# sadPororo/AD-YOLO

Hardware: AMD Instinct MI355X
Metric: train-step audio-sec/s (4ch, se-resnet34+adyolo) (higher is better)
Workload: dtype f32; 1 GPU; se-resnet34 + adyolo loss, synthetic 4ch 24kHz 60s clips, bs=64 per GPU, 12 classes, features+fwd+loss+bwd+allreduce+Adam; global_batch=64, parallelism=dp1

## Files before the change

ad-yolo_amd/_lib.py:

```python
import ctypes
import os

_HERE = os.path.dirname(os.path.abspath(__file__))
LIB_PATH = os.environ.get("ADYOLO_LIB") or os.path.join(_HERE, "libadyolo_hip.so")

P = ctypes.c_void_p
I = ctypes.c_int
L = ctypes.c_long
F = ctypes.c_float
U64 = ctypes.c_uint64

SIGNATURES = {
    "adyolo_abi_version": (I, []),
    "adyolo_last_error": (ctypes.c_char_p, []),
    "adyolo_feat_stft_mel": (I, [P] * 8 + [I, I] + [P] * 4 + [I, I, I, P]),
    "adyolo_feat_finish": (I, [P] * 4 + [I, I, I, P]),
    "adyolo_feat_gcc_phat": (I, [P] * 6 + [I, I, I, I, P]),
    "adyolo_nchw_to_nhwc8": (I, [P, P, I, I, I, I, P]),
    "adyolo_pack_w3x3": (I, [P, P, P, I, I, I, P]),
    "adyolo_conv3x3_tiles": (I, [I] * 3),
    "adyolo_conv3x3_fwd": (I, [P] * 13 + [I] * 7 + [P]),
    "adyolo_wino_pack_w": (I, [P, P, P, I, I, I, P]),
    "adyolo_wino_pack_many": (I, [P, I, I, I, P]),
    "adyolo_wino_tiles": (I, [I] * 3),
    "adyolo_wino_fwd": (I, [P] * 13 + [I] * 7 + [P]),
    "adyolo_wino4_pack_w": (I, [P, P, P, I, I, I, P]),
    "adyolo_wino4_pack_many": (I, [P, I, I, I, P]),
    "adyolo_wino4_tiles": (I, [I] * 3),
    "adyolo_wino4_fwd": (I, [P] * 13 + [I] * 7 + [P]),
    "adyolo_wino4_fwd_form": (I, [I] * 3),
    "adyolo_wino4_last_form": (I, []),
    "adyolo_set_switches": (I, [I]),
    "adyolo_wino4_wgrad_slabs": (I, [I] * 5),
    "adyolo_wino4_wgrad": (I, [P] * 7 + [I] * 6 + [P]),
    "adyolo_wino_wgrad_slabs": (I, [I] * 5),
    "adyolo_wino_wgrad": (I, [P] * 7 + [I] * 6 + [P]),
    "adyolo_conv3x3_wgrad_slabs": (I, [I] * 5),
    "adyolo_conv3x3_wgrad": (I, [P] * 6 + [I] * 6 + [P]),
    "adyolo_wgrad_plan": (I, [I] * 6 + [P]),
    "adyolo_conv_fwd_plan": (I, [I] * 9 + [P]),
    "adyolo_gemm": (I, [P] * 5 + [I] * 10 + [P]),
    "adyolo_gemm_plan": (I, [I] * 8 + [P, P, P]),
    "adyolo_gemm_batched": (I, [P] * 3 + [I] * 10 + [L] * 6 + [F, I, P]),
    "adyolo_colsum": (I, [P, P, P, I, I, I, I, P]),
    "adyolo_bn_stats": (I, [P] * 7 + [I, I, I, F, F, P]),
    "adyolo_bn_stats_tiles": (I, [P] * 11 + [I, I, I, I, F, F, P]),
    "adyolo_bn_eval_stats": (I, [P] * 4 + [I, F, P]),
    "adyolo_bn_scale_shift": (I, [P] * 6 + [I, P]),
    "adyolo_affine_nhwc": (I, [P] * 4 + [L, I, P]),
    "adyolo_bn_bwd_reduce": (I, [P] * 7 + [L, I, P]),
    "adyolo_bn_bwd_tiles": (I, [P, P, P, P, I, I, P]),
    "adyolo_bn_bwd_apply": (I, [P] * 12 + [L, I, I, F, P]),
    "adyolo_bn_persample": (I, [P, P, P, I, I, I, P]),
    "adyolo_bn_finish": (I, [P] * 10 + [I, I, I, F, F, P]),
    "adyolo_se_fc_fwd": (I, [P] * 10 + [I, I, I, I, P]),
    "adyolo_relu_mask_words": (L, [I, I, I]),
    "adyolo_se_tail_fwd": (I, [P] * 9 + [I, I, I, P]),
    "adyolo_se_tail_fwd_pool_ok": (I, [I, I, I]),
    "adyolo_se_tail_fwd_pool": (I, [P] * 9 + [I, I, I, I, P]),
    "adyolo_se_tail_bwd_reduce": (I, [P] * 9 + [I, I, I, P]),
    "adyolo_se_tail_bwd_tiles": (I, [P, P, P, I, I, I, P]),
    "adyolo_se_fc_bwd_words": (L, [I, I]),
    "adyolo_se_fc_bwd": (I, [P] * 16 + [I, I, I, I, P]),
    "adyolo_se_tail_bwd_apply": (I, [P] * 13 + [I, I, I, F, P]),
    "adyolo_se_tail_bwd_reduce_pooled": (I, [P] * 8 + [I, I, I, I, P]),
    "adyolo_se_tail_bwd_apply_pooled": (I, [P] * 13 + [I, I, I, I, F, P]),
    "adyolo_avgpool2_fwd": (I, [P, P, I, I, I, I, P]),
    "adyolo_avgpool2_bwd": (I, [P, P, I, I, I, I, P]),
    "adyolo_add": (I, [P, P, P, L, P]),
    "adyolo_mul": (I, [P, P, P, L, P]),
    "adyolo_scale_dev": (I, [P, P, P, L, P]),
    "adyolo_sap_fwd": (I, [P] * 5 + [I, I, I, P]),
    "adyolo_sap_bwd": (I, [P] * 8 + [I, I, I, P]),
    "adyolo_gru_fwd": (I, [P] * 6 + [I, I, P]),
    "adyolo_gru_bwd": (I, [P] * 6 + [I, I, P]),
    "adyolo_ln_tanh_fwd": (I, [P] * 4 + [L, I, F, P]),
    "adyolo_ln_tanh_bwd": (I, [P] * 8 + [L, I, F, P]),
    "adyolo_dropout_mask": (I, [P, L, F, U64, U64, P]),
    "adyolo_dropout_apply": (I, [P, P, L, F, U64, U64, P]),
    "adyolo_dropout_apply_dev": (I, [P, P, L, F, U64, U64, P, P]),
    "adyolo_counter_add": (I, [P, U64, P]),
    "adyolo_loss_workspace_words": (L, [I, I, I, I]),
    "adyolo_loss_fwd_bwd": (I, [P] * 6 + [I] * 7 + [P, P, F, F, F, F, P]),
    "adyolo_loss_phase": (I, [P] * 6 + [I] * 7 + [P, P, F, F, F, F, I, L, P]),
    "adyolo_loss_per_clip_workspace_words": (L, [I, I, I, I]),
    "adyolo_loss_per_clip": (I, [P] * 7 + [I] * 6 + [L, P, P, F, F, F, P]),
    "adyolo_loss_accumulate": (I, [P, P, I, P, P]),
    "adyolo_yolo_decode": (I, [P, P, L, I, I, I, I, F, F, F, P]),
    "adyolo_yolo_select_workspace_words": (L, [L, I, I]),
    "adyolo_yolo_select": (I, [P] * 4 + [L, I, I, F, F, F, F, I, P]),
    "adyolo_seld_score_workspace_words": (L, [L, I, I, I]),
    "adyolo_seld_score": (I, [P, I, L, P, L, I] + [P] * 5 + [I, I, I, I, ctypes.c_double, P, P, P, P]),
    "adyolo_act_fwd": (I, [P, P, L, I, I, P]),
    "adyolo_act_bwd": (I, [P, P, P, L, I, I, P]),
    "adyolo_seddoa_loss": (I, [P] * 5 + [L, I, I, I, F, F, P]),
    "adyolo_adpit_loss": (I, [P] * 5 + [L, I, P]),
    "adyolo_classwise_decode": (I, [P, P, L, I, I, P]),
    "adyolo_classwise_select_workspace_words": (L, [L, I, I]),
    "adyolo_classwise_select": (I, [P] * 4 + [L, I, I, F, F, P]),
    "adyolo_tta_merge_workspace_words": (L, [L, I]),
    "adyolo_tta_collect": (I, [P, L, P, P, P, P, P, L, I, I, I, I, ctypes.c_uint, P]),
    "adyolo_tta_merge": (I, [P, P, P, P, L, P, P, L, I, I, I, F, I, P]),
    "adyolo_conv_gemm": (I, [P, P, P, P] + [I] * 13 + [P]),
    "adyolo_conv_gemm_plan": (I, [I] * 13 + [P]),
    "adyolo_pack_wk": (I, [P, P, I, I, I, I, I, P]),
    "adyolo_maxpool3_fwd": (I, [P, P, P, I, I, I, I, P]),
    "adyolo_maxpool3_bwd": (I, [P, P, P, I, I, I, I, P]),
    "adyolo_affine_relu_nhwc": (I, [P] * 4 + [L, I, P]),
    "adyolo_relu_bwd": (I, [P, P, P, L, P]),
    "adyolo_axpby": (I, [P, P, P, F, F, L, P]),
    "adyolo_dropout_axpby": (I, [P, P, P, L, F, U64, U64, P, F, F, P]),
    "adyolo_swish_fwd": (I, [P, P, L, P]),
    "adyolo_swish_bwd": (I, [P, P, P, L, P]),
    "adyolo_glu_fwd": (I, [P, P, L, I, P]),
    "adyolo_glu_bwd": (I, [P, P, P, L, I, P]),
    "adyolo_dwconv3_fwd": (I, [P] * 4 + [I, I, I, I, I, P]),
    "adyolo_dwconv3_wgrad": (I, [P] * 6 + [I, I, I, I, P]),
    "adyolo_softmax_fwd": (I, [P, P, L, I, F, P]),
    "adyolo_softmax_bwd": (I, [P, P, P, L, I, F, P]),
# ... 93 lines not shown
```

ad-yolo_amd/csrc/norm.hip:

```cpp
#include "common.hpp"

namespace adyolo {

#ifndef ADYOLO_EW_NT
#define ADYOLO_EW_NT 3
#endif
__device__ __forceinline__ float4 ew_ld(const float4 *p) {
#if ADYOLO_EW_NT & 1
    const f32x4 v = __builtin_nontemporal_load(reinterpret_cast<const f32x4 *>(p));
    return make_float4(v[0], v[1], v[2], v[3]);
#else
    return *p;
#endif
}
__device__ __forceinline__ void ew_st(float4 *p, const float4 &v) {
#if ADYOLO_EW_NT & 2
    const f32x4 t = {v.x, v.y, v.z, v.w};
    __builtin_nontemporal_store(t, reinterpret_cast<f32x4 *>(p));
#else
    *p = v;
#endif
}


// ... 535 lines not shown
        ew_st(&dc4[i], o);
        if (dr4) dr4[i] = g;
    };
    if (INV) {
        load_params((int)threadIdx.x % c4n);
        const long step = (long)gridDim.x * 256 * EW_U;
        for (long i0 = (long)blockIdx.x * 256 * EW_U + threadIdx.x; i0 < hw4; i0 += step) {
            float4 d[EW_U], cv[EW_U];
            bool px[EW_U], py[EW_U], pz[EW_U], pw[EW_U];
#pragma unroll
            for (int u = 0; u < EW_U; ++u) {
                const long i = i0 + u * 256;
                if (i < hw4) {
                    if (POOLED) {
                        const int pix = (int)(i >> c4shift), y = pix / W, x = pix - y * W;
                        const float4 g4 = de4[(((size_t)(y >> 1) * (W >> 1) + (x >> 1)) << c4shift) + (i & (c4n - 1))];
                        d[u] = make_float4(0.25f * g4.x, 0.25f * g4.y, 0.25f * g4.z, 0.25f * g4.w);
                    } else {
                        d[u] = ew_ld(&de4[i]);
                    }
                    cv[u] = ew_ld(&c4[i]);
                    if (mask) {
                        mask_bits4(mask, base + i, px[u], py[u], pz[u], pw[u]);
                    } else {
                        const float4 ev = e4[i];
                        px[u] = ev.x > 0.f; py[u] = ev.y > 0.f; pz[u] = ev.z > 0.f; pw[u] = ev.w > 0.f;
                    }
                }
            }
#pragma unroll
            for (int u = 0; u < EW_U; ++u) {
                const long i = i0 + u * 256;
                if (i < hw4) {
                    one(i, d[u], cv[u], px[u], py[u], pz[u], pw[u]);
                    if (POOLED && deo4) ew_st(&deo4[i], d[u]);
                }
            }
        }
    } else {
        for (long i = (long)blockIdx.x * blockDim.x + threadIdx.x; i < hw4; i += (long)gridDim.x * blockDim.x) {
            load_params((int)(i % c4n));
            bool px, py, pz, pw;
            if (mask) {
                mask_bits4(mask, base + i, px, py, pz, pw);
            } else {
                const float4 ev = e4[i];
                px = ev.x > 0.f; py = ev.y > 0.f; pz = ev.z > 0.f; pw = ev.w > 0.f;
            }
            one(i, de4[i], c4[i], px, py, pz, pw);
        }
    }
}

__global__ __launch_bounds__(256) void avgpool2_fwd_kernel(const float *__restrict__ x, float *__restrict__ y,
                                                           int H, int W, int c4n, long total4) {
    const int Ho = H >> 1, Wo = W >> 1;
    for (long i = (long)blockIdx.x * blockDim.x + threadIdx.x; i < total4; i += (long)gridDim.x * blockDim.x) {
        const int cx = (int)(i % c4n);
        long p = i / c4n;
        const int wo = (int)(p % Wo);
        p /= Wo;
        const int ho = (int)(p % Ho);
        const long n = p / Ho;
        const float4 *src = reinterpret_cast<const float4 *>(x) + (((size_t)n * H + 2 * ho) * W + 2 * wo) * c4n + cx;
        const float4 a = ew_ld(src), b = ew_ld(src + c4n), c = ew_ld(src + (size_t)W * c4n), d = ew_ld(src + (size_t)W * c4n + c4n);
        reinterpret_cast<float4 *>(y)[i] = make_float4(0.25f * (a.x + b.x + c.x + d.x), 0.25f * (a.y + b.y + c.y + d.y),
                                                       0.25f * (a.z + b.z + c.z + d.z), 0.25f * (a.w + b.w + c.w + d.w));
    }
}
__global__ __launch_bounds__(256) void avgpool2_bwd_kernel(const float *__restrict__ dy, float *__restrict__ dx,
                                                           int H, int W, int c4n, long total4) {
    const int Ho = H >> 1, Wo = W >> 1;
    for (long i = (long)blockIdx.x * blockDim.x + threadIdx.x; i < total4; i += (long)gridDim.x * blockDim.x) {
        const int cx = (int)(i % c4n);
        long p = i / c4n;
        const int w = (int)(p % W);
        p /= W;
        const int h = (int)(p % H);
        const long n = p / H;
        const float4 g = reinterpret_cast<const float4 *>(dy)[(((size_t)n * Ho + (h >> 1)) * Wo + (w >> 1)) * c4n + cx];
        ew_st(&reinterpret_cast<float4 *>(dx)[i], make_float4(0.25f * g.x, 0.25f * g.y, 0.25f * g.z, 0.25f * g.w));
    }
}

static inline int ew_grid(long n4) {
    long g = (n4 + 255) / 256;
    return (int)(g > 8192 ? 8192 : (g < 1 ? 1 : g));
}
static inline bool chan_ok(int C) { return C >= 4 && C <= 1024 && (C % 4) == 0 && (256 % (C / 4)) == 0; }
static inline int pick_G(int N, int HW) {
    int G = 1024 / N;
    if (G < 1) G = 1;
    const int need = (HW + 63) / 64;
    if (G > need) G = need;
    return G;
}

}

using namespace adyolo;

extern "C" int adyolo_bn_stats(const float *x, float *ssum, float *mean, float *invstd, float *running_mean,
                               float *running_var, float *partial, int N, int HW, int C, float momentum, float eps,
                               void *stream) {
    ADYOLO_REQUIRE(x && mean && invstd && partial && N > 0 && HW > 0, ADYOLO_EINVAL, "bn_stats: bad arguments");
    ADYOLO_REQUIRE(chan_ok(C) && N <= 1024, ADYOLO_ENOSUP, "bn_stats: unsupported C=%d or N=%d", C, N);
// ... 258 lines not shown
    hipLaunchKernelGGL(se_fc_bwd_sample_kernel, dim3(N), dim3(256), 0, as_stream(stream), sg, sgx, ssum, gamma, beta,
                       mean, invstd, pooled, hid, s, w1, w2, dpool, part, HW, C, Cr);
    int rc = check_launch("se_fc_bwd_sample");
    if (rc) return rc;
    const long P = adyolo_se_fc_bwd_words(C, Cr);
    return adyolo_colsum(part, packed, colsum_ws, N, (int)P, (int)P, 0, stream);
}

extern "C" int adyolo_se_tail_bwd_apply(const float *de, const float *e, const uint64_t *mask, const float *c,
                                        const float *gamma, const float *mean, const float *invstd, const float *s,
                                        const float *dpool, const float *sdd, const float *sddx, float *dc, float *dr,
                                        int N, int HW, int C, float count_scale, void *stream) {
    ADYOLO_REQUIRE(de && (e || mask) && c && gamma && mean && invstd && s && dpool && sdd && sddx && dc && N > 0 &&
                       HW > 0 && C % 4 == 0 && count_scale >= 1.f,
                   ADYOLO_EINVAL, "se_tail_bwd_apply: bad arguments");
    const float inv_r = (float)(1.0 / ((double)N * (double)HW * (double)count_scale));
    const long hw4 = (long)HW * (C / 4);
    const bool inv = 256 % (C / 4) == 0;
    int gx = ew_grid(inv ? cdiv(hw4, (long)EW_U) : hw4);
    if ((long)gx * N > 16384) gx = (int)(16384 / N > 0 ? 16384 / N : 1);
    if (inv)
        hipLaunchKernelGGL(se_tail_bwd_apply_kernel<true>, dim3(gx, N), dim3(256), 0, as_stream(stream), de, e, c, gamma,
                           mean, invstd, s, dpool, sdd, sddx, dc, dr, reinterpret_cast<const unsigned long long *>(mask),
                           hw4, C / 4, 1.0f / (float)HW, inv_r);
    else
        hipLaunchKernelGGL(se_tail_bwd_apply_kernel<false>, dim3(gx, N), dim3(256), 0, as_stream(stream), de, e, c, gamma,
                           mean, invstd, s, dpool, sdd, sddx, dc, dr, reinterpret_cast<const unsigned long long *>(mask),
                           hw4, C / 4, 1.0f / (float)HW, inv_r);
    return check_launch("se_tail_bwd_apply");
}

extern "C" int adyolo_se_tail_bwd_apply_pooled(const float *dpooled, const uint64_t *mask, const float *c, const float *gamma,
                                               const float *mean, const float *invstd, const float *s, const float *dpool,
                                               const float *sdd, const float *sddx, float *dc, float *dr, float *de_out, int N,
                                               int H, int W, int C, float count_scale, void *stream) {
    ADYOLO_REQUIRE(dpooled && mask && c && gamma && mean && invstd && s && dpool && sdd && sddx && dc && N > 0 && H > 0 && W > 0 &&
                       count_scale >= 1.f,
                   ADYOLO_EINVAL, "se_tail_bwd_apply_pooled: bad arguments");
    ADYOLO_REQUIRE(adyolo_se_tail_fwd_pool_ok(H, W, C), ADYOLO_ENOSUP, "se_tail_bwd_apply_pooled: unsupported shape H=%d W=%d C=%d",
                   H, W, C);
    const int HW = H * W, c4n = C / 4;
    int c4shift = 0;
    while ((1 << c4shift) < c4n) ++c4shift;
    const float inv_r = (float)(1.0 / ((double)N * (double)HW * (double)count_scale));
    const long hw4 = (long)HW * c4n;
    int gx = ew_grid(cdiv(hw4, (long)EW_U));
    if ((long)gx * N > 16384) gx = (int)(16384 / N > 0 ? 16384 / N : 1);
    hipLaunchKernelGGL((se_tail_bwd_apply_kernel<true, true>), dim3(gx, N), dim3(256), 0, as_stream(stream), dpooled,
                       (const float *)nullptr, c, gamma, mean, invstd, s, dpool, sdd, sddx, dc, dr,
                       reinterpret_cast<const unsigned long long *>(mask), hw4, c4n, 1.0f / (float)HW, inv_r, W, c4shift, de_out);
    return check_launch("se_tail_bwd_apply_pooled");
}

extern "C" int adyolo_avgpool2_fwd(const float *x, float *y, int N, int H, int W, int C, void *stream) {
    ADYOLO_REQUIRE(x && y && N > 0 && H > 0 && W > 0 && H % 2 == 0 && W % 2 == 0 && C % 4 == 0, ADYOLO_EINVAL,
                   "avgpool2_fwd: H, W must be even and C %% 4 == 0");
    const long total4 = (long)N * (H / 2) * (W / 2) * (C / 4);
    hipLaunchKernelGGL(avgpool2_fwd_kernel, dim3(ew_grid(total4)), dim3(256), 0, as_stream(stream), x, y, H, W, C / 4,
                       total4);
    return check_launch("avgpool2_fwd");
}
extern "C" int adyolo_avgpool2_bwd(const float *dy, float *dx, int N, int H, int W, int C, void *stream) {
    ADYOLO_REQUIRE(dy && dx && N > 0 && H > 0 && W > 0 && H % 2 == 0 && W % 2 == 0 && C % 4 == 0, ADYOLO_EINVAL,
                   "avgpool2_bwd: H, W must be even and C %% 4 == 0");
    const long total4 = (long)N * H * W * (C / 4);
    hipLaunchKernelGGL(avgpool2_bwd_kernel, dim3(ew_grid(total4)), dim3(256), 0, as_stream(stream), dy, dx, H, W, C / 4,
                       total4);
    return check_launch("avgpool2_bwd");
}
```

ad-yolo_amd/functional.py:

```python
import os
from typing import NamedTuple

import torch

from . import ops

FUSE_BNBWD = os.environ.get("ADYOLO_FUSE_BNBWD", "1") != "0"
FUSE_POOL = os.environ.get("ADYOLO_FUSE_POOL", "1") != "0"
FUSE_POOL_BWD = os.environ.get("ADYOLO_FUSE_POOL_BWD", "1") != "0"


class BlockLink:

    def __init__(self):
        self.cc = self.mean2 = self.invstd2 = self.tiles = self.ebits = None
        self.affine = self.stem_bn = None
        self.prepooled = None


class BlockArgs(NamedTuple):
    bn1: object
    bn2: object
    bnd: object = None
    link_in: object = None
    link_out: object = None
    in_affine: tuple = None
    stem_holder: object = None
    packs: tuple = None
    pool_next: bool = False


def _c(t):
    return t if t.is_contiguous() else t.contiguous()


_CONST = {}


def _const(value, shape, device):
    key = (float(value), tuple(shape), str(device))
    t = _CONST.get(key)
    if t is None:
        t = torch.full(tuple(shape), float(value), dtype=torch.float32, device=device)
        _CONST[key] = t
    return t


class GradSink:

    def __init__(self):
        self.views = None
        self.notify = None
        self.step = 4

    def begin(self, flat, reducer=None):
        self.views = {p.data_ptr(): (i, p.grad) for i, p in enumerate(flat.params)}
        self.notify = reducer.notify if (reducer is not None and reducer.active) else None

    def end(self):
        self.views = self.notify = None

    def view(self, ptr, shape=None):
# ... 215 lines not shown
        if ctx.link_out is not None:
            link_out.cc, link_out.mean2, link_out.invstd2, link_out.tiles = cc, mean2, invstd2, None
            link_out.ebits = ebits
        ctx.training, ctx.pool, ctx.has_down = training, pool and not prepooled, wd is not None
        ctx.pool_out = (h, w_) if pool_out else None
        ctx.in_hw = (x.shape[1], x.shape[2])
        ctx.p_aff = p_aff
        ctx.stem_holder = args.stem_holder
        ctx.dgrad_packs = (wpk1d, wpk2d)
        ctx.ptrs = (w1.data_ptr(), g1.data_ptr(), b1.data_ptr(), w2.data_ptr(),
                    (fb2.data_ptr(), fw2.data_ptr(), fb1.data_ptr(), fw1.data_ptr(), b2.data_ptr(), g2.data_ptr()))
        ctx.wshapes = (tuple(w1.shape), tuple(w2.shape))
        ctx.down_ptrs = (wd.data_ptr(), gd.data_ptr(), bd.data_ptr(), tuple(wd.shape)) if wd is not None else None
        tensors = [p, a, scale1, shift1, cc, None if pool_out else e, ebits, g1, mean1, invstd1, g2, b2, mean2, invstd2, ssum2,
                   pooled, hid, s, fw1, fw2]
        names = ["p", "a", "scale1", "shift1", "cc", "e", "ebits", "g1", "mean1", "invstd1", "g2", "b2", "mean2", "invstd2",
                 "ssum2", "pooled", "hid", "s", "fw1", "fw2"]
        if wd is not None:
            tensors += [q, wd, gd, meand, invstdd]
            names += ["q", "wd", "gd", "meand", "invstdd"]
        ctx.saved_names = names
        ctx.save_for_backward(*tensors)
        return e

    @staticmethod
    def backward(ctx, de):
        if not ctx.training:
            raise NotImplementedError("backward through eval-mode BatchNorm is not part of the hot path")
        t = ctx.saved_tensors
        (p, a, scale1, shift1, cc, e, ebits, g1, mean1, invstd1, g2, b2, mean2, invstd2, ssum2, pooled, hid, s, fw1,
         fw2) = t[:20]
        wpk1d, wpk2d = ctx.dgrad_packs
        n, h, w_, cin = p.shape
        c = cc.shape[-1]
        de = _c(de)
        pooled_hw = None
        if ctx.pool_out is not None and FUSE_POOL_BWD:
            pooled_hw = ctx.pool_out
        elif ctx.pool_out is not None:
            de = ops.avgpool2_bwd(de, ctx.pool_out[0], ctx.pool_out[1])
        tiles = None
        if ctx.link_out is not None and ctx.link_out.tiles is not None:
            tiles, ctx.link_out.tiles = ctx.link_out.tiles, None
        pw1, pg1, pb1, pw2, pse = ctx.ptrs
        vse = SINK.span(pse)
        vw1, vw2 = SINK.view(pw1, ctx.wshapes[0]), SINK.view(pw2, ctx.wshapes[1])
        vg1, vb1 = SINK.view(pg1), SINK.view(pb1)
        sunk = vse is not None and vw1 is not None and vw2 is not None and vg1 is not None and vb1 is not None
        if not sunk:
            vse = vw1 = vw2 = vg1 = vb1 = None
        de_full = None
        if pooled_hw is not None and not ctx.has_down:
            de_full = torch.empty(n, pooled_hw[0], pooled_hw[1], c, dtype=torch.float32, device=de.device)
        dc, dr, dg2, db2, dfw1, dfb1, dfw2, dfb2 = ops.se_tail_bwd(de, e, cc, g2, b2, mean2, invstd2, ssum2, pooled,
                                                                   hid, s, fw1, fw2,
                                                                   want_dr=ctx.has_down, tile_stats=tiles,
                                                                   mask=ebits, packed_out=vse, pooled_hw=pooled_hw,
                                                                   de_out=de_full)
        if pooled_hw is not None:
            de = de_full
        dw2 = ops.conv3x3_wgrad(a, dc, c, in_affine=(scale1, shift1), out=vw2)
        if FUSE_BNBWD:
            dbb, st = ops.conv3x3(dc, wpk2d, c, want_stats=True, stat_bn=(a, mean1, invstd1))
            da, dg1, db1 = ops.bn_bwd(dbb, a, g1, mean1, invstd1, relu_mask=True, tile_stats=st, out_dgamma=vg1,
                                      out_dbeta=vb1)
        else:
            dbb = ops.conv3x3(dc, wpk2d, c)
            da, dg1, db1 = ops.bn_bwd(dbb, a, g1, mean1, invstd1, relu_mask=True, out_dgamma=vg1, out_dbeta=vb1)
        dw1 = ops.conv3x3_wgrad(p, da, cin, in_affine=ctx.p_aff, out=vw1)
        if sunk:
            SINK.done(*pse)
            SINK.done(pw2, pg1, pb1, pw1)
            dw1 = dg1 = db1 = dw2 = dg2 = db2 = dfw1 = dfb1 = dfw2 = dfb2 = None
        dwd = dgd = dbd = None
        if ctx.has_down:
            q, wd, gd, meand, invstdd = t[20:25]
            pwd, pgd, pbd, wdshape = ctx.down_ptrs
            vwd, vgd, vbd = SINK.view(pwd, (wdshape[0], wdshape[1])), SINK.view(pgd), SINK.view(pbd)
            dsunk = sunk and vwd is not None and vgd is not None and vbd is not None
            if not dsunk:
                vwd = vgd = vbd = None
            dq, dgd, dbd = ops.bn_bwd(dr, q, gd, meand, invstdd, relu_mask=False, out_dgamma=vgd, out_dbeta=vbd)
            rows = n * h * w_
            dwd = ops.gemm(dq, p, c, cin, rows, c, cin, trans_a=True, trans_b=True,
                           splits=ops.wgrad_splits(c, cin, rows), out=vwd).view(c, cin, 1, 1)
            if dsunk:
                SINK.done(pwd, pgd, pbd)
                dwd = dgd = dbd = None
            addend = ops.gemm(dq, wd, rows, cin, c, c, cin, trans_b=True).view(n, h, w_, cin)
            amask = None
        else:
            addend, amask = de, (ebits if ebits is not None else e)
        lk, holder = ctx.link_in, ctx.stem_holder
        if lk is not None:
            dp, lk.tiles = ops.conv3x3(da, wpk1d, cin, addend=addend, addend_mask=amask, want_stats=True,
                                       stat_bn=(lk.cc, lk.mean2, lk.invstd2), stat_mask=lk.ebits if lk.ebits is not None else p)
        elif not ctx.has_down and holder is not None and holder.stem_bn is not None:
            dp, holder.tiles = ops.conv3x3(da, wpk1d, cin, addend=addend, addend_mask=amask, want_stats=True, stat_bn=holder.stem_bn)
        else:
            dp = ops.conv3x3(da, wpk1d, cin, addend=addend, addend_mask=amask)
        dx = ops.avgpool2_bwd(dp, ctx.in_hw[0], ctx.in_hw[1]) if ctx.pool else dp
        return (dx, None, None, None, dw1, dg1, db1, dw2, dg2, db2, dfw1, dfb1, dfw2, dfb2, dwd, dgd, dbd)


class SAPFn(torch.autograd.Function):

    @staticmethod
    def forward(ctx, x, w, b):
        bsz, t, f, c = x.shape
        y, attn = ops.sap_fwd(x.view(bsz * t, f, c), w.view(-1), b)
        ctx.bias = b
        ctx.save_for_backward(x, w, attn)
        return y.view(bsz, t, c)

    @staticmethod
    def backward(ctx, dy):
        x, w, attn = ctx.saved_tensors
        bsz, t, f, c = x.shape
        sunk = SINK.params(w, ctx.bias) if (ctx.needs_input_grad[1] and ctx.needs_input_grad[2]) else None
        dx, dw, db = ops.sap_bwd(_c(dy).view(bsz * t, c), x.view(bsz * t, f, c), w.view(-1), attn,
                                 out_dw=sunk[0].view(-1) if sunk is not None else None, out_db=sunk[1] if sunk is not None else None)
        if sunk is not None:
            SINK.done_params(w, ctx.bias)
            return dx.view(bsz, t, f, c), None, None
        return dx.view(bsz, t, f, c), dw.view_as(w), db


class BiGRULayerFn(torch.autograd.Function):

    @staticmethod
    def forward(ctx, x, wih_f, whh_f, bih_f, bhh_f, wih_r, whh_r, bih_r, bhh_r, save):
        bsz, t, cin = x.shape
        rows = bsz * t
        x2 = x.view(rows, cin)
        gx = torch.empty(rows, 768, dtype=torch.float32, device=x.device)
# ... 484 lines not shown
```

ad-yolo_amd/ops.py:

```python
import ctypes
import os

import numpy as np
import torch

from . import _lib

_c = _lib.call
NULL = ctypes.c_void_p(0)


def _p(t):
    if t is None:
        return NULL
    return ctypes.c_void_p(t.data_ptr())


def _stream():
    return ctypes.c_void_p(torch.cuda.current_stream().cuda_stream)


def _chk(*ts):
    for t in ts:
        if t is None:
# ... 457 lines not shown
def bn_eval_stats(running_mean, running_var, eps=1e-5):
    _chk(running_mean, running_var)
    c = running_mean.numel()
    mean, invstd = _new(running_mean, c), _new(running_mean, c)
    _c("adyolo_bn_eval_stats", _p(running_mean), _p(running_var), _p(mean), _p(invstd), c, eps, _stream())
    return mean, invstd


def bn_scale_shift(gamma, beta, mean, invstd):
    _chk(gamma, beta, mean, invstd)
    c = gamma.numel()
    scale, shift = _new(gamma, c), _new(gamma, c)
    _c("adyolo_bn_scale_shift", _p(gamma), _p(beta), _p(mean), _p(invstd), _p(scale), _p(shift), c, _stream())
    return scale, shift


def affine(x, scale, shift):
    _chk(x, scale, shift)
    c = x.shape[-1]
    y = torch.empty_like(x)
    _c("adyolo_affine_nhwc", _p(x), _p(scale), _p(shift), _p(y), x.numel() // c, c, _stream())
    return y


def bn_bwd(dy, x, gamma, mean, invstd, relu_mask=False, tile_stats=None, out_dgamma=None, out_dbeta=None,
           want_dx_colsum=False):
    _chk(dy, x, gamma, mean, invstd)
    c = x.shape[-1]
    rows = x.numel() // c
    sdy = out_dbeta if out_dbeta is not None else _new(x, c)
    sdyx = out_dgamma if out_dgamma is not None else _new(x, c)
    if tile_stats is not None:
        _c("adyolo_bn_bwd_tiles", _p(tile_stats), _p(sdy), _p(sdyx), _p(_new(tile_stats, 2, 256, c)), tile_stats.shape[1], c,
           _stream())
    else:
        partial = _new(x, 2 * 1024 * c)
        _c("adyolo_bn_bwd_reduce", _p(dy), _p(x), _p(mean), _p(invstd), _p(sdy), _p(sdyx), _p(partial), rows, c,
           _stream())
    dx = torch.empty_like(x)
    colsum = part = None
    if want_dx_colsum:
        colsum, part = _new(x, c), _new(x, 8192, c)
    a_sdy, a_sdyx, cs = sdy, sdyx, 1.0
    if EXACT.on:
        glob = EXACT.all_reduce(torch.stack([sdy, sdyx]))
        a_sdy, a_sdyx, cs = glob[0], glob[1], float(EXACT.world)
    _c("adyolo_bn_bwd_apply", _p(dy), _p(x), _p(gamma), _p(mean), _p(invstd), _p(a_sdy), _p(a_sdyx), _p(dx), NULL, NULL,
       _p(colsum), _p(part), rows, c, int(relu_mask), cs, _stream())
    if want_dx_colsum:
        return dx, sdyx, sdy, colsum
    return dx, sdyx, sdy


def se_fc_fwd(ssum, scale, shift, w1, b1, w2, b2, hw):
    _chk(ssum, scale, shift, w1, b1, w2, b2)
    n, c = ssum.shape
    cr = w1.shape[0]
    pooled, hid, s = _new(ssum, n, c), _new(ssum, n, cr), _new(ssum, n, c)
    _c("adyolo_se_fc_fwd", _p(ssum), _p(scale), _p(shift), _p(w1), _p(b1), _p(w2), _p(b2), _p(pooled), _p(hid), _p(s),
       n, hw, c, cr, _stream())
    return pooled, hid, s


def se_tail_pool_ok(h, w, ch):
    return bool(_lib.load().adyolo_se_tail_fwd_pool_ok(int(h), int(w), int(ch)))


def se_tail_fwd(c_t, r_t, scale, shift, s, want_mask=False, r_affine=None, pool_hw=None):
    _chk(c_t, r_t, scale, shift, s)
    n, ch = c_t.shape[0], c_t.shape[-1]
    hw = c_t.numel() // (n * ch)
    mask = None
    if want_mask:
        words = _lib.load().adyolo_relu_mask_words(n, hw, ch)
        if words > 0:
            mask = torch.empty(words, dtype=torch.int64, device=c_t.device)
    rs, rt = r_affine if r_affine is not None else (None, None)
    if pool_hw is not None:
        h, w = pool_hw
        if want_mask and mask is None:
            raise _lib.AdyoloHipError("se_tail_fwd(pool_hw=): the shape has no mask bits")
        pooled = _new(c_t, n, h // 2, w // 2, ch)
        _c("adyolo_se_tail_fwd_pool", _p(c_t), _p(r_t), _p(scale), _p(shift), _p(s), _p(rs), _p(rt), _p(pooled), _p(mask), n, h, w,
           ch, _stream())
        return pooled, mask
    e = torch.empty_like(c_t)
    _c("adyolo_se_tail_fwd", _p(c_t), _p(r_t), _p(scale), _p(shift), _p(s), _p(rs), _p(rt), _p(e), _p(mask), n, hw, ch,
       _stream())
    return (e, mask) if want_mask else e


def se_tail_bwd(de, e, c_t, gamma, beta, mean, invstd, ssum, pooled, hid, s, w1, w2, want_dr=True, tile_stats=None,
                mask=None, packed_out=None, pooled_hw=None, de_out=None):
    _chk(de, e, c_t, gamma, beta, mean, invstd, ssum, pooled, hid, s, w1, w2, de_out)
    if pooled_hw is not None and mask is None:
        raise _lib.AdyoloHipError("se_tail_bwd(pooled_hw=) needs the ReLU-mask bits")
    n, ch = c_t.shape[0], c_t.shape[-1]
    hw = c_t.numel() // (n * ch)
    cr = w1.shape[0]
    sg, sgx = _new(c_t, n, ch), _new(c_t, n, ch)
    if tile_stats is not None:
        _c("adyolo_se_tail_bwd_tiles", _p(tile_stats), _p(sg), _p(sgx), n, tile_stats.shape[1] // n, ch, _stream())
    else:
        partial = _new(c_t, 2 * 1024 * ch)
        if pooled_hw is not None:
            _c("adyolo_se_tail_bwd_reduce_pooled", _p(de), _p(mask), _p(c_t), _p(mean), _p(invstd), _p(sg), _p(sgx), _p(partial),
               n, pooled_hw[0], pooled_hw[1], ch, _stream())
        else:
            _c("adyolo_se_tail_bwd_reduce", _p(de), _p(e), _p(mask), _p(c_t), _p(mean), _p(invstd), _p(sg), _p(sgx), _p(partial),
               n, hw, ch, _stream())
    pw = 2 * ch * cr + cr + 3 * ch
    part, cws = _new(c_t, n, pw), _new(c_t, 1024, pw)
    packed = packed_out if packed_out is not None else _new(c_t, pw)
    dpool = _new(c_t, n, ch)
    _c("adyolo_se_fc_bwd", _p(sg), _p(sgx), _p(ssum), _p(gamma), _p(beta), _p(mean), _p(invstd), _p(pooled), _p(hid),
       _p(s), _p(w1), _p(w2), _p(dpool), _p(part), _p(packed), _p(cws), n, hw, ch, cr, _stream())
    o = 0
    db2 = packed[o:o + ch]; o += ch
    dw2 = packed[o:o + ch * cr].view(ch, cr); o += ch * cr
    db1 = packed[o:o + cr]; o += cr
    dw1 = packed[o:o + cr * ch].view(cr, ch); o += cr * ch
    sdd = packed[o:o + ch]; o += ch
    sddx = packed[o:o + ch]
    dgamma, dbeta = sddx, sdd
    dc = torch.empty_like(c_t)
    dr = torch.empty_like(c_t) if want_dr else None
    a_sdd, a_sddx, cs = sdd, sddx, 1.0
    if EXACT.on:
        glob = EXACT.all_reduce(torch.stack([sdd, sddx]))
        a_sdd, a_sddx, cs = glob[0], glob[1], float(EXACT.world)
    if pooled_hw is not None:
        _c("adyolo_se_tail_bwd_apply_pooled", _p(de), _p(mask), _p(c_t), _p(gamma), _p(mean), _p(invstd), _p(s), _p(dpool),
           _p(a_sdd), _p(a_sddx), _p(dc), _p(dr), _p(de_out), n, pooled_hw[0], pooled_hw[1], ch, cs, _stream())
    else:
        _c("adyolo_se_tail_bwd_apply", _p(de), _p(e), _p(mask), _p(c_t), _p(gamma), _p(mean), _p(invstd), _p(s), _p(dpool),
           _p(a_sdd), _p(a_sddx), _p(dc), _p(dr), n, hw, ch, cs, _stream())
    return dc, dr, dgamma, dbeta, dw1, db1, dw2, db2


def avgpool2(x):
    _chk(x)
    n, h, w, c = x.shape
    y = _new(x, n, h // 2, w // 2, c)
    _c("adyolo_avgpool2_fwd", _p(x), _p(y), n, h, w, c, _stream())
    return y


def avgpool2_bwd(dy, h, w):
    _chk(dy)
    n, c = dy.shape[0], dy.shape[3]
    dx = _new(dy, n, h, w, c)
    _c("adyolo_avgpool2_bwd", _p(dy), _p(dx), n, h, w, c, _stream())
    return dx


def sap_fwd(x, w, b):
    _chk(x, w, b)
    r, f, c = x.shape
    y, attn = _new(x, r, c), _new(x, r, f)
    _c("adyolo_sap_fwd", _p(x), _p(w), _p(b), _p(y), _p(attn), r, f, c, _stream())
    return y, attn


def sap_bwd(dy, x, w, attn, out_dw=None, out_db=None):
    _chk(dy, x, w, attn)
    r, f, c = x.shape
    dx = torch.empty_like(x)
    dw = out_dw if out_dw is not None else _zeros(x, c)
    db = out_db if out_db is not None else _zeros(x, 1)
    partial = _new(x, 1024 * 260)
    _c("adyolo_sap_bwd", _p(dy), _p(x), _p(w), _p(attn), _p(dx), _p(dw), _p(db), _p(partial), r, f, c, _stream())
    return dx, dw, db


def gru_fwd(gx, whh, bhh, save):
    _chk(gx, whh, bhh)
    b, t = gx.shape[0], gx.shape[1]
    out = _new(gx, b, t, 256)
    gates = _new(gx, b, t, 2, 4, 128) if save else None
    hprev = _new(gx, b, t, 2, 128) if save else None
    _c("adyolo_gru_fwd", _p(gx), _p(whh), _p(bhh), _p(out), _p(gates), _p(hprev), b, t, _stream())
    return out, gates, hprev


# ... 1250 lines not shown
```

include/adyolo_hip.h:

```cpp
#ifndef ADYOLO_HIP_H
#define ADYOLO_HIP_H

#include <stddef.h>
#include <stdint.h>

#ifdef __cplusplus
extern "C" {
#endif

#define ADYOLO_ABI_VERSION 4
#define ADYOLO_EINVAL (-1)
#define ADYOLO_ENOSUP (-2)

int         adyolo_abi_version(void);
const char *adyolo_last_error(void);

int adyolo_feat_stft_mel(const float *audio, const int64_t *clip_offset, const float *twiddle,
                         const int32_t *chunk_mel, const int32_t *chunk_start, const int32_t *chunk_len,
                         const int32_t *chunk_off, const float *mel_w, int n_chunks, int n_mel_w,
                         const float *scaler_mean, const float *scaler_rstd, float *out, float *chan_max, int B,
                         int n_samples, int layout, void *stream);
int adyolo_feat_finish(float *out, const float *chan_max, const float *scaler_mean,
                       const float *scaler_rstd, int B, int T, int layout, void *stream);

// ... 69 lines not shown
int adyolo_bn_persample(const float *tile_stats, float *ps0, float *ps1, int N, int G, int C, void *stream);
int adyolo_bn_finish(const float *ps0, const float *ps1, float *mean, float *invstd, float *running_mean,
                     float *running_var, const float *gamma, const float *beta, float *scale, float *shift, int N,
                     int HW, int C, float momentum, float eps, void *stream);
int adyolo_bn_eval_stats(const float *running_mean, const float *running_var, float *mean,
                         float *invstd, int C, float eps, void *stream);
int adyolo_bn_scale_shift(const float *gamma, const float *beta, const float *mean,
                          const float *invstd, float *scale, float *shift, int C, void *stream);
int adyolo_affine_nhwc(const float *x, const float *scale, const float *shift, float *y, long rows,
                       int C, void *stream);
int adyolo_bn_bwd_reduce(const float *dy, const float *x, const float *mean, const float *invstd,
                         float *sdy, float *sdyx, float *partial, long rows, int C, void *stream);
int adyolo_bn_bwd_tiles(const float *tile_stats, float *sdy, float *sdyx, float *partial , int tiles, int C,
                        void *stream);
int adyolo_bn_bwd_apply(const float *dy, const float *x, const float *gamma, const float *mean,
                        const float *invstd, const float *sdy, const float *sdyx, float *dx,
                        float *dgamma, float *dbeta, float *dx_colsum ,
                        float *colsum_partial , long rows, int C, int relu_mask,
                        float count_scale ,
                        void *stream);

int adyolo_se_fc_fwd(const float *ssum, const float *scale, const float *shift, const float *w1,
                     const float *b1, const float *w2, const float *b2, float *pooled, float *hid,
                     float *s, int N, int HW, int C, int Cr, void *stream);
long adyolo_relu_mask_words(int N, int HW, int C);
int adyolo_se_tail_fwd(const float *c, const float *r, const float *scale, const float *shift,
                       const float *s, const float *r_scale , const float *r_shift , float *e,
                       uint64_t *mask , int N, int HW, int C, void *stream);
int adyolo_se_tail_fwd_pool_ok(int H, int W, int C);
int adyolo_se_tail_fwd_pool(const float *c, const float *r, const float *scale, const float *shift, const float *s,
                            const float *r_scale , const float *r_shift , float *pooled,
                            uint64_t *mask , int N, int H, int W, int C, void *stream);
int adyolo_se_tail_bwd_reduce(const float *de, const float *e, const uint64_t *mask , const float *c,
                              const float *mean, const float *invstd, float *sg, float *sgx, float *partial, int N,
                              int HW, int C, void *stream);
int adyolo_se_tail_bwd_tiles(const float *tile_stats, float *sg, float *sgx, int N, int G, int C, void *stream);
long adyolo_se_fc_bwd_words(int C, int Cr);
int adyolo_se_fc_bwd(const float *sg, const float *sgx, const float *ssum, const float *gamma,
                     const float *beta, const float *mean, const float *invstd, const float *pooled,
                     const float *hid, const float *s, const float *w1, const float *w2, float *dpool,
                     float *part , float *packed , float *colsum_ws , int N,
                     int HW, int C, int Cr, void *stream);
int adyolo_se_tail_bwd_reduce_pooled(const float *dpooled, const uint64_t *mask, const float *c, const float *mean,
                                     const float *invstd, float *sg, float *sgx, float *partial, int N, int H, int W, int C,
                                     void *stream);
int adyolo_se_tail_bwd_apply_pooled(const float *dpooled, const uint64_t *mask, const float *c, const float *gamma,
                                    const float *mean, const float *invstd, const float *s, const float *dpool,
                                    const float *sdd, const float *sddx, float *dc, float *dr ,
                                    float *de_out , int N, int H, int W, int C, float count_scale, void *stream);
int adyolo_se_tail_bwd_apply(const float *de, const float *e, const uint64_t *mask , const float *c,
                             const float *gamma, const float *mean, const float *invstd, const float *s,
                             const float *dpool, const float *sdd, const float *sddx, float *dc,
                             float *dr, int N, int HW, int C, float count_scale , void *stream);

int adyolo_avgpool2_fwd(const float *x, float *y, int N, int H, int W, int C, void *stream);
int adyolo_avgpool2_bwd(const float *dy, float *dx, int N, int H, int W, int C, void *stream);
int adyolo_add(const float *a, const float *b, float *y, long n, void *stream);
int adyolo_scale_dev(const float *a, const float *scalar_dev, float *y, long n, void *stream);

int adyolo_sap_fwd(const float *x, const float *w, const float *b, float *y, float *attn, int R,
                   int F, int C, void *stream);
int adyolo_sap_bwd(const float *dy, const float *x, const float *w, const float *attn, float *dx,
                   float *dw, float *db, float *partial, int R, int F, int C, void *stream);

int adyolo_gru_fwd(const float *gx, const float *whh, const float *bhh, float *out, float *gates,
                   float *hprev, int B, int T, void *stream);
int adyolo_gru_bwd(const float *dout, const float *gates, const float *hprev, const float *whh,
                   float *dgx, float *dgh, int B, int T, void *stream);
int adyolo_ln_tanh_fwd(const float *x, const float *gamma, const float *beta, float *y, long R,
                       int C, float eps, void *stream);
int adyolo_ln_tanh_bwd(const float *dy, const float *x, const float *y, const float *gamma,
                       float *dx, float *dgamma, float *dbeta, float *partial, long R, int C,
                       float eps, void *stream);
int adyolo_dropout_mask(float *mask, long n, float p, uint64_t seed, uint64_t offset, void *stream);
int adyolo_dropout_apply(const float *x, float *y, long n, float p, uint64_t seed, uint64_t offset, void *stream);
int adyolo_dropout_apply_dev(const float *x, float *y, long n, float p, uint64_t seed, uint64_t offset,
                             const uint64_t *offset_dev, void *stream);
int adyolo_counter_add(uint64_t *counter, uint64_t inc, void *stream);
int adyolo_mul(const float *a, const float *b, float *y, long n, void *stream);

long adyolo_loss_workspace_words(int BT, int G, int A, int M);
int  adyolo_loss_fwd_bwd(const float *logit, const float *target, float *ws, float *loss,
                         float *dlogit, float *dist, int B, int T, int Gaz, int Gel, int A, int C,
                         int M, const float *thr_host, const float *gains_host, float grid_az,
                         float grid_el, float g_overlap, float grad_scale, void *stream);
int  adyolo_loss_phase(const float *logit, const float *target, float *ws, float *loss,
                       float *dlogit, float *dist, int B, int T, int Gaz, int Gel, int A, int C,
                       int M, const float *thr_host, const float *gains_host, float grid_az,
                       float grid_el, float g_overlap, float grad_scale, int phases, long na_total, void *stream);

long adyolo_loss_per_clip_workspace_words(int B, int T, int G, int A);
int  adyolo_loss_per_clip(const float *logit, const float *target, const int *row_start, float *ws, float *loss,
                          int *valid, float *acc, int B, int T, int Gaz, int Gel, int A, int C, long cap,
                          const float *thr_host, const float *gains_host, float grid_az, float grid_el,
                          float g_overlap, void *stream);
int  adyolo_loss_accumulate(const float *loss, const int *valid, int n, float *acc, void *stream);

int adyolo_yolo_decode(const float *logit, float *out, long n_frames, int Gaz, int Gel, int A, int C,
                       float grid_az, float grid_el, float g_overlap, void *stream);

#define ADYOLO_SELECT_PLAIN 0
#define ADYOLO_SELECT_CONN  1
#define ADYOLO_SELECT_SOFT  2
#define ADYOLO_SELECT_MAX_N 1024
long adyolo_yolo_select_workspace_words(long n_frames, int n_anchor, int C);
int  adyolo_yolo_select(const float *dec, float *ws, float *rows, int *frame_counts, long n_frames, int n_anchor, int C,
// ... 208 lines not shown
```

Baseline: 36560 audio-s/s.

## Fuse downsample-BN backward stats into SE tail apply, skip materialising dr

For SE blocks with a downsample projection, the SE-tail backward apply kernel now also accumulates per-tile sums of the masked gradient and of its product with the normalised projection input. This replaces writing the full residual gradient tensor and a separate BN-backward reduction pass over it. A new masked BN-backward apply kernel recomputes the residual gradient on the fly from de and the ReLU mask bits. The aim is to save one full-size write and read of dr plus a reduction pass. The cost is extra loads of q in the fused kernel and a somewhat different summation order.

```diff
diff --git a/ad-yolo_amd/_lib.py b/ad-yolo_amd/_lib.py
--- a/ad-yolo_amd/_lib.py
+++ b/ad-yolo_amd/_lib.py
@@ -65,6 +65,9 @@
     "adyolo_se_tail_bwd_apply": (I, [P] * 13 + [I, I, I, F, P]),
     "adyolo_se_tail_bwd_reduce_pooled": (I, [P] * 8 + [I, I, I, I, P]),
     "adyolo_se_tail_bwd_apply_pooled": (I, [P] * 13 + [I, I, I, I, F, P]),
+    "adyolo_se_tail_bwd_apply_proj_tiles": (L, [I, I, I]),
+    "adyolo_se_tail_bwd_apply_proj": (I, [P] * 15 + [I, I, I, F, P]),
+    "adyolo_bn_bwd_apply_masked": (I, [P] * 9 + [L, I, F, P]),
     "adyolo_avgpool2_fwd": (I, [P, P, I, I, I, I, P]),
     "adyolo_avgpool2_bwd": (I, [P, P, I, I, I, I, P]),
     "adyolo_add": (I, [P, P, P, L, P]),
diff --git a/ad-yolo_amd/csrc/norm.hip b/ad-yolo_amd/csrc/norm.hip
--- a/ad-yolo_amd/csrc/norm.hip
+++ b/ad-yolo_amd/csrc/norm.hip
@@ -611,6 +611,126 @@
     }
 }
 
+__global__ __launch_bounds__(256) void se_tail_bwd_apply_proj_kernel(
+    const float *__restrict__ de, const float *__restrict__ c, const float *__restrict__ q,
+    const float *__restrict__ gamma, const float *__restrict__ mean, const float *__restrict__ invstd,
+    const float *__restrict__ s, const float *__restrict__ dpool, const float *__restrict__ sdd,
+    const float *__restrict__ sddx, const float *__restrict__ meand, const float *__restrict__ invstdd,
+    float *__restrict__ dc, const unsigned long long *__restrict__ mask, float *__restrict__ tile_stats, unsigned hw4, int rows,
+    int chunk, int c4n, float invHW, float invR) {
+    __shared__ float4 sred[2][256];
+    const float4 *de4 = reinterpret_cast<const float4 *>(de), *c4 = reinterpret_cast<const float4 *>(c);
+    const float4 *q4 = reinterpret_cast<const float4 *>(q);
+    const float4 *s4 = reinterpret_cast<const float4 *>(s), *dp4 = reinterpret_cast<const float4 *>(dpool);
+    float4 *dc4 = reinterpret_cast<float4 *>(dc);
+    const int cx = (int)threadIdx.x % c4n;
+    const float4 ga = reinterpret_cast<const float4 *>(gamma)[cx];
+    const float4 m = reinterpret_cast<const float4 *>(mean)[cx];
+    const float4 is = reinterpret_cast<const float4 *>(invstd)[cx];
+    const float4 a = reinterpret_cast<const float4 *>(sdd)[cx];
+    const float4 b = reinterpret_cast<const float4 *>(sddx)[cx];
+    const float4 md = reinterpret_cast<const float4 *>(meand)[cx];
+    const float4 isd = reinterpret_cast<const float4 *>(invstdd)[cx];
+    float4 u = make_float4(0.f, 0.f, 0.f, 0.f), v = u;
+    const int rbeg = blockIdx.x * chunk, rend = min(rows, rbeg + chunk);
+    const unsigned iend = (unsigned)rend * c4n;
+    for (unsigned i0 = (unsigned)rbeg * c4n + threadIdx.x; i0 < iend; i0 += 256 * EW_U) {
+        float4 d[EW_U], cv[EW_U], qv[EW_U], sv[EW_U], dp[EW_U];
+        bool px[EW_U], py[EW_U], pz[EW_U], pw[EW_U];
+#pragma unroll
+        for (int k = 0; k < EW_U; ++k) {
+            const unsigned i = i0 + k * 256;
+            if (i < iend) {
+                const unsigned n = i / hw4;
+                d[k] = ew_ld(&de4[i]);
+                cv[k] = ew_ld(&c4[i]);
+                qv[k] = ew_ld(&q4[i]);
+                sv[k] = s4[n * c4n + cx];
+                dp[k] = dp4[n * c4n + cx];
+                mask_bits4(mask, i, px[k], py[k], pz[k], pw[k]);
+            }
+        }
+#pragma unroll
+        for (int k = 0; k < EW_U; ++k) {
+            const unsigned i = i0 + k * 256;
+            if (i < iend) {
+                float4 g, o;
+                g.x = px[k] ? d[k].x : 0.f;
+                g.y = py[k] ? d[k].y : 0.f;
+                g.z = pz[k] ? d[k].z : 0.f;
+                g.w = pw[k] ? d[k].w : 0.f;
+                o.x = ga.x * is.x * (g.x * sv[k].x + dp[k].x * invHW - a.x * invR - (cv[k].x - m.x) * is.x * b.x * invR);
+                o.y = ga.y * is.y * (g.y * sv[k].y + dp[k].y * invHW - a.y * invR - (cv[k].y - m.y) * is.y * b.y * invR);
+                o.z = ga.z * is.z * (g.z * sv[k].z + dp[k].z * invHW - a.z * invR - (cv[k].z - m.z) * is.z * b.z * invR);
+                o.w = ga.w * is.w * (g.w * sv[k].w + dp[k].w * invHW - a.w * invR - (cv[k].w - m.w) * is.w * b.w * invR);
+                ew_st(&dc4[i], o);
+                const float4 t = make_float4(g.x * (qv[k].x - md.x) * isd.x, g.y * (qv[k].y - md.y) * isd.y,
+                                             g.z * (qv[k].z - md.z) * isd.z, g.w * (qv[k].w - md.w) * isd.w);
+                u.x += g.x; u.y += g.y; u.z += g.z; u.w += g.w;
+                v.x += t.x; v.y += t.y; v.z += t.z; v.w += t.w;
+            }
+        }
+    }
+    sred[0][threadIdx.x] = u;
+    sred[1][threadIdx.x] = v;
+    __syncthreads();
+    if ((int)threadIdx.x < c4n) {
+        float4 t0 = make_float4(0.f, 0.f, 0.f, 0.f), t1 = t0;
+        for (int k = threadIdx.x; k < 256; k += c4n) {
+            const float4 w0 = sred[0][k], w1 = sred[1][k];
+            t0.x += w0.x; t0.y += w0.y; t0.z += w0.z; t0.w += w0.w;
+            t1.x += w1.x; t1.y += w1.y; t1.z += w1.z; t1.w += w1.w;
+        }
+        float4 *ts4 = reinterpret_cast<float4 *>(tile_stats);
+        ts4[(size_t)blockIdx.x * c4n + threadIdx.x] = t0;
+        ts4[(size_t)gridDim.x * c4n + (size_t)blockIdx.x * c4n + threadIdx.x] = t1;
+    }
+}
+
+__global__ __launch_bounds__(256) void bn_bwd_apply_masked_kernel(
+    const float *__restrict__ de, const unsigned long long *__restrict__ mask, const float *__restrict__ x,
+    const float *__restrict__ gamma, const float *__restrict__ mean, const float *__restrict__ invstd,
+    const float *__restrict__ sdy, const float *__restrict__ sdyx, float *__restrict__ dx, long n4, int c4n, float invR) {
+    const int cx = (int)threadIdx.x % c4n;
+    const float4 g = reinterpret_cast<const float4 *>(gamma)[cx];
+    const float4 m = reinterpret_cast<const float4 *>(mean)[cx];
+    const float4 is = reinterpret_cast<const float4 *>(invstd)[cx];
+    const float4 a = reinterpret_cast<const float4 *>(sdy)[cx];
+    const float4 b = reinterpret_cast<const float4 *>(sdyx)[cx];
+    const float4 *de4 = reinterpret_cast<const float4 *>(de), *x4 = reinterpret_cast<const float4 *>(x);
+    float4 *dx4 = reinterpret_cast<float4 *>(dx);
+    const long step = (long)gridDim.x * 256 * EW_U;
+    for (long i0 = (long)blockIdx.x * 256 * EW_U + threadIdx.x; i0 < n4; i0 += step) {
+        float4 d[EW_U], xv[EW_U];
+#pragma unroll
+        for (int k = 0; k < EW_U; ++k) {
+            const long i = i0 + k * 256;
+            if (i < n4) {
+                bool px, py, pz, pw;
+                d[k] = ew_ld(&de4[i]);
+                xv[k] = ew_ld(&x4[i]);
+                mask_bits4(mask, (size_t)i, px, py, pz, pw);
+                if (!px) d[k].x = 0.f;
+                if (!py) d[k].y = 0.f;
+                if (!pz) d[k].z = 0.f;
+                if (!pw) d[k].w = 0.f;
+            }
+        }
+#pragma unroll
+        for (int k = 0; k < EW_U; ++k) {
+            const long i = i0 + k * 256;
+            if (i < n4) {
+                float4 o;
+                o.x = g.x * is.x * (d[k].x - a.x * invR - (xv[k].x - m.x) * is.x * b.x * invR);
+                o.y = g.y * is.y * (d[k].y - a.y * invR - (xv[k].y - m.y) * is.y * b.y * invR);
+                o.z = g.z * is.z * (d[k].z - a.z * invR - (xv[k].z - m.z) * is.z * b.z * invR);
+                o.w = g.w * is.w * (d[k].w - a.w * invR - (xv[k].w - m.w) * is.w * b.w * invR);
+                ew_st(&dx4[i], o);
+            }
+        }
+    }
+}
+
 __global__ __launch_bounds__(256) void avgpool2_fwd_kernel(const float *__restrict__ x, float *__restrict__ y,
                                                            int H, int W, int c4n, long total4) {
     const int Ho = H >> 1, Wo = W >> 1;
@@ -975,6 +1095,48 @@
     return check_launch("se_tail_bwd_apply_pooled");
 }
 
+static int proj_apply_G(int N, int HW, int C) {
+    if (N <= 0 || HW <= 0 || !chan_ok(C)) return 0;
+    const long hw4 = (long)HW * (C / 4), rows = (long)N * HW;
+    if (hw4 % 64 != 0 || rows * (C / 4) >= (1L << 31)) return 0;
+    const long G = (rows + 63) / 64;
+    return (int)(G > 1024 ? 1024 : G);
+}
+extern "C" long adyolo_se_tail_bwd_apply_proj_tiles(int N, int HW, int C) { return proj_apply_G(N, HW, C); }
+
+extern "C" int adyolo_se_tail_bwd_apply_proj(const float *de, const uint64_t *mask, const float *c, const float *q,
+                                             const float *gamma, const float *mean, const float *invstd, const float *s,
+                                             const float *dpool, const float *sdd, const float *sddx, const float *meand,
+                                             const float *invstdd, float *dc, float *tile_stats, int N, int HW, int C,
+                                             float count_scale, void *stream) {
+    ADYOLO_REQUIRE(de && mask && c && q && gamma && mean && invstd && s && dpool && sdd && sddx && meand && invstdd && dc &&
+                       tile_stats && N > 0 && HW > 0 && count_scale >= 1.f,
+                   ADYOLO_EINVAL, "se_tail_bwd_apply_proj: bad arguments");
+    const int G = proj_apply_G(N, HW, C);
+    ADYOLO_REQUIRE(G > 0, ADYOLO_ENOSUP, "se_tail_bwd_apply_proj: unsupported shape N=%d HW=%d C=%d", N, HW, C);
+    const float inv_r = (float)(1.0 / ((double)N * (double)HW * (double)count_scale));
+    const int rows = N * HW, chunk = (rows + G - 1) / G;
+    hipLaunchKernelGGL(se_tail_bwd_apply_proj_kernel, dim3(G), dim3(256), 0, as_stream(stream), de, c, q, gamma, mean, invstd,
+                       s, dpool, sdd, sddx, meand, invstdd, dc, reinterpret_cast<const unsigned long long *>(mask), tile_stats,
+                       (unsigned)(HW * (C / 4)), rows, chunk, C / 4, 1.0f / (float)HW, inv_r);
+    return check_launch("se_tail_bwd_apply_proj");
+}
+
+extern "C" int adyolo_bn_bwd_apply_masked(const float *de, const uint64_t *mask, const float *x, const float *gamma,
+                                          const float *mean, const float *invstd, const float *sdy, const float *sdyx,
+                                          float *dx, long rows, int C, float count_scale, void *stream) {
+    ADYOLO_REQUIRE(de && mask && x && gamma && mean && invstd && sdy && sdyx && dx && rows > 0 && count_scale >= 1.f,
+                   ADYOLO_EINVAL, "bn_bwd_apply_masked: bad arguments");
+    ADYOLO_REQUIRE(chan_ok(C) && (rows * (C / 4)) % 64 == 0, ADYOLO_ENOSUP,
+                   "bn_bwd_apply_masked: unsupported shape rows=%ld C=%d", rows, C);
+    const float inv_r = (float)(1.0 / ((double)rows * (double)count_scale));
+    const long n4 = rows * (C / 4);
+    hipLaunchKernelGGL(bn_bwd_apply_masked_kernel, dim3(ew_grid(cdiv(n4, (long)EW_U))), dim3(256), 0, as_stream(stream), de,
+                       reinterpret_cast<const unsigned long long *>(mask), x, gamma, mean, invstd, sdy, sdyx, dx, n4, C / 4,
+                       inv_r);
+    return check_launch("bn_bwd_apply_masked");
+}
+
 extern "C" int adyolo_avgpool2_fwd(const float *x, float *y, int N, int H, int W, int C, void *stream) {
     ADYOLO_REQUIRE(x && y && N > 0 && H > 0 && W > 0 && H % 2 == 0 && W % 2 == 0 && C % 4 == 0, ADYOLO_EINVAL,
                    "avgpool2_fwd: H, W must be even and C %% 4 == 0");
diff --git a/ad-yolo_amd/functional.py b/ad-yolo_amd/functional.py
--- a/ad-yolo_amd/functional.py
+++ b/ad-yolo_amd/functional.py
@@ -8,6 +8,7 @@
 FUSE_BNBWD = os.environ.get("ADYOLO_FUSE_BNBWD", "1") != "0"
 FUSE_POOL = os.environ.get("ADYOLO_FUSE_POOL", "1") != "0"
 FUSE_POOL_BWD = os.environ.get("ADYOLO_FUSE_POOL_BWD", "1") != "0"
+FUSE_PROJ = os.environ.get("ADYOLO_FUSE_PROJ", "1") != "0"
 
 
 class BlockLink:
@@ -329,11 +330,15 @@
         de_full = None
         if pooled_hw is not None and not ctx.has_down:
             de_full = torch.empty(n, pooled_hw[0], pooled_hw[1], c, dtype=torch.float32, device=de.device)
+        proj_bn = None
+        if (ctx.has_down and FUSE_PROJ and ebits is not None and pooled_hw is None and not ops.EXACT.on
+                and ops.se_tail_bwd_proj_tiles(n, h * w_, c) > 0):
+            proj_bn = (t[20], t[23], t[24])
         dc, dr, dg2, db2, dfw1, dfb1, dfw2, dfb2 = ops.se_tail_bwd(de, e, cc, g2, b2, mean2, invstd2, ssum2, pooled,
                                                                    hid, s, fw1, fw2,
                                                                    want_dr=ctx.has_down, tile_stats=tiles,
                                                                    mask=ebits, packed_out=vse, pooled_hw=pooled_hw,
-                                                                   de_out=de_full)
+                                                                   de_out=de_full, proj_bn=proj_bn)
         if pooled_hw is not None:
             de = de_full
         dw2 = ops.conv3x3_wgrad(a, dc, c, in_affine=(scale1, shift1), out=vw2)
@@ -357,7 +362,10 @@
             dsunk = sunk and vwd is not None and vgd is not None and vbd is not None
             if not dsunk:
                 vwd = vgd = vbd = None
-            dq, dgd, dbd = ops.bn_bwd(dr, q, gd, meand, invstdd, relu_mask=False, out_dgamma=vgd, out_dbeta=vbd)
+            if proj_bn is not None:
+                dq, dgd, dbd = ops.bn_bwd_masked(de, ebits, q, gd, meand, invstdd, dr, out_dgamma=vgd, out_dbeta=vbd)
+            else:
+                dq, dgd, dbd = ops.bn_bwd(dr, q, gd, meand, invstdd, relu_mask=False, out_dgamma=vgd, out_dbeta=vbd)
             rows = n * h * w_
             dwd = ops.gemm(dq, p, c, cin, rows, c, cin, trans_a=True, trans_b=True,
                            splits=ops.wgrad_splits(c, cin, rows), out=vwd).view(c, cin, 1, 1)
diff --git a/ad-yolo_amd/ops.py b/ad-yolo_amd/ops.py
--- a/ad-yolo_amd/ops.py
+++ b/ad-yolo_amd/ops.py
@@ -533,6 +533,19 @@
     return dx, sdyx, sdy
 
 
+def bn_bwd_masked(de, mask, x, gamma, mean, invstd, tile_stats, out_dgamma=None, out_dbeta=None):
+    _chk(de, x, gamma, mean, invstd, tile_stats)
+    c = x.shape[-1]
+    rows = x.numel() // c
+    sdy = out_dbeta if out_dbeta is not None else _new(x, c)
+    sdyx = out_dgamma if out_dgamma is not None else _new(x, c)
+    _c("adyolo_se_tail_bwd_tiles", _p(tile_stats), _p(sdy), _p(sdyx), 1, tile_stats.shape[1], c, _stream())
+    dx = torch.empty_like(x)
+    _c("adyolo_bn_bwd_apply_masked", _p(de), _p(mask), _p(x), _p(gamma), _p(mean), _p(invstd), _p(sdy), _p(sdyx), _p(dx), rows, c,
+       1.0, _stream())
+    return dx, sdyx, sdy
+
+
 def se_fc_fwd(ssum, scale, shift, w1, b1, w2, b2, hw):
     _chk(ssum, scale, shift, w1, b1, w2, b2)
     n, c = ssum.shape
@@ -545,6 +558,10 @@
 
 def se_tail_pool_ok(h, w, ch):
     return bool(_lib.load().adyolo_se_tail_fwd_pool_ok(int(h), int(w), int(ch)))
+
+
+def se_tail_bwd_proj_tiles(n, hw, ch):
+    return int(_lib.load().adyolo_se_tail_bwd_apply_proj_tiles(int(n), int(hw), int(ch)))
 
 
 def se_tail_fwd(c_t, r_t, scale, shift, s, want_mask=False, r_affine=None, pool_hw=None):
@@ -572,7 +589,7 @@
 
 
 def se_tail_bwd(de, e, c_t, gamma, beta, mean, invstd, ssum, pooled, hid, s, w1, w2, want_dr=True, tile_stats=None,
-                mask=None, packed_out=None, pooled_hw=None, de_out=None):
+                mask=None, packed_out=None, pooled_hw=None, de_out=None, proj_bn=None):
     _chk(de, e, c_t, gamma, beta, mean, invstd, ssum, pooled, hid, s, w1, w2, de_out)
     if pooled_hw is not None and mask is None:
         raise _lib.AdyoloHipError("se_tail_bwd(pooled_hw=) needs the ReLU-mask bits")
@@ -605,12 +622,20 @@
     sddx = packed[o:o + ch]
     dgamma, dbeta = sddx, sdd
     dc = torch.empty_like(c_t)
-    dr = torch.empty_like(c_t) if want_dr else None
+    dr = torch.empty_like(c_t) if (want_dr and proj_bn is None) else None
     a_sdd, a_sddx, cs = sdd, sddx, 1.0
     if EXACT.on:
         glob = EXACT.all_reduce(torch.stack([sdd, sddx]))
         a_sdd, a_sddx, cs = glob[0], glob[1], float(EXACT.world)
-    if pooled_hw is not None:
+    if proj_bn is not None:
+        q, meand, invstdd = proj_bn
+        _chk(q, meand, invstdd)
+        if pooled_hw is not None or mask is None or q.shape != c_t.shape:
+            raise _lib.AdyoloHipError("se_tail_bwd(proj_bn=) needs the mask bits, an un-pooled output and q shaped like c")
+        dr = _new(c_t, 2, se_tail_bwd_proj_tiles(n, hw, ch), ch)
+        _c("adyolo_se_tail_bwd_apply_proj", _p(de), _p(mask), _p(c_t), _p(q), _p(gamma), _p(mean), _p(invstd), _p(s), _p(dpool),
+           _p(a_sdd), _p(a_sddx), _p(meand), _p(invstdd), _p(dc), _p(dr), n, hw, ch, cs, _stream())
+    elif pooled_hw is not None:
         _c("adyolo_se_tail_bwd_apply_pooled", _p(de), _p(mask), _p(c_t), _p(gamma), _p(mean), _p(invstd), _p(s), _p(dpool),
            _p(a_sdd), _p(a_sddx), _p(dc), _p(dr), _p(de_out), n, pooled_hw[0], pooled_hw[1], ch, cs, _stream())
     else:
diff --git a/include/adyolo_hip.h b/include/adyolo_hip.h
--- a/include/adyolo_hip.h
+++ b/include/adyolo_hip.h
@@ -145,6 +145,14 @@
                              const float *gamma, const float *mean, const float *invstd, const float *s,
                              const float *dpool, const float *sdd, const float *sddx, float *dc,
                              float *dr, int N, int HW, int C, float count_scale , void *stream);
+long adyolo_se_tail_bwd_apply_proj_tiles(int N, int HW, int C);
+int adyolo_se_tail_bwd_apply_proj(const float *de, const uint64_t *mask, const float *c, const float *q, const float *gamma,
+                                  const float *mean, const float *invstd, const float *s, const float *dpool,
+                                  const float *sdd, const float *sddx, const float *meand, const float *invstdd, float *dc,
+                                  float *tile_stats, int N, int HW, int C, float count_scale, void *stream);
+int adyolo_bn_bwd_apply_masked(const float *de, const uint64_t *mask, const float *x, const float *gamma, const float *mean,
+                               const float *invstd, const float *sdy, const float *sdyx, float *dx, long rows, int C,
+                               float count_scale, void *stream);
 
 int adyolo_avgpool2_fwd(const float *x, float *y, int N, int H, int W, int C, void *stream);
 int adyolo_avgpool2_bwd(const float *dy, float *dx, int N, int H, int W, int C, void *stream);
```

Result: no change. 36650 audio-s/s, median of 6 (+0.3%).
